# ISAE-PNX/SaDVIO

Measured on AMD Instinct MI355X. Metric: BA iterations/sec (ms/solve in ms_per_solve), 20-KF/8k-landmark window, higher is better.
Workload: dtype f64; 1 GPU; synthetic 20 KF x 8000 landmarks x 40000 reprojection factors (pixel), GN 10 iters (LM step attempts, early exits disabled); windows_per_gpu=1, parallelism=single window, n_kf=20, n_lmk=8000, n_obs=40000, reduced_dim=114

## Files before the change

### sadvio_amd/csrc/kernels.h

```cpp
#pragma once
#include "ba_types.h"
#include "device_math.h"
#include "chol16.h"

namespace sadvio {

struct DevPtrs {
    const WinDev* win;
    const Tile* tiles;
    const double* kf_T0;
    const int* kf_fidx;
    double* xp; double* xv; double* xba; double* xbg;
    long long xp_stride, xv_stride, xl_stride;
    const double* kf_vel; const double* kf_ba; const double* kf_bg;
    const double* cam_K; const double* cam_T; const double* cam_isig;
    const double* lmk_p; double* xl; double* s_lmk;
    const unsigned char* lmk_const;
    const int* lmk_ob; const int* lmk_oe;
    const int* obs_kf; const int* obs_cam; const double* obs_meas;
    const unsigned char* obs_slot;
    const int* tile_kf;
    const int* tile_lmk;
    const int* tile_row;
    const int4* pre_lane;
// ... 260 lines not shown

struct ObsLin {
    double r[2], Jp[12], Jl[6];
    double rho;
    int row;
    int slot;
    bool valid;
    bool counted;
};

struct ObsPre {
    int slot, craw;
    double m[3];
};
template <int FACTOR>
__device__ __forceinline__ ObsPre obs_prefetch(const DevPtrs& P, int o) {
    ObsPre q;
    q.slot = P.obs_slot[o];
    q.craw = P.obs_cam[o];
    if (FACTOR == 0) { const double* m = P.obs_meas + 2 * (long long)o; q.m[0] = m[0]; q.m[1] = m[1]; q.m[2] = 0.0; }
    else { const double* m = P.obs_meas + 3 * (long long)o; q.m[0] = m[0]; q.m[1] = m[1]; q.m[2] = m[2]; }
    return q;
}

template <int FACTOR, bool RARE>
__device__ __forceinline__ void lane_linearize(const DevPtrs& P, const double* poseTab, const double* camTab,
                                               const int* rowTab, int cam_base, const ObsPre& ob, const double* pw, bool keep_jl,
                                               bool lcounted, ObsLin& L) {
    const int slot = ob.slot;
    const int craw = ob.craw;
    const int cam = craw < 0 ? 0 : craw - cam_base;
    const double* tab = poseTab + slot * POSE_TAB;
    const double* ct = camTab + cam * 17;
    L.slot = slot;
    L.row = rowTab[slot];
    if (RARE && craw < 0) {
        const int code = -1 - craw;
        const SparseDev& f = P.sparse[code >> 1];
        p2l_pseudo_obs<true>(tab, pw, f.delta, f.W, code & 1, L.r, L.Jp, L.Jl);
        L.rho = L.r[0] * L.r[0] + L.r[1] * L.r[1];
        if (L.row < 0) {
#pragma unroll
            for (int i = 0; i < 12; i++) L.Jp[i] = 0.0;
        }
        if (!keep_jl) {
#pragma unroll
            for (int i = 0; i < 6; i++) L.Jl[i] = 0.0;
        }
        L.counted = (L.row >= 0) || lcounted;
        return;
    }
    if (FACTOR == 0) {
        pixel_factor<true>(tab, ct, ct + 4, pw, ob.m[0], ob.m[1], ct[16], L.r, L.Jp, L.Jl);
    } else {
        double b[3] = {ob.m[0], ob.m[1], ob.m[2]};
        angular_factor<true>(tab, ct + 4, pw, b, ct[16], L.r, L.Jp, L.Jl);
    }
    L.rho = L.r[0] * L.r[0] + L.r[1] * L.r[1];
    if (RARE) {
        double sc;
        L.rho = huber_rho(P.o.huber_a, L.rho, sc);
        if (sc != 1.0) {
            L.r[0] *= sc; L.r[1] *= sc;
#pragma unroll
            for (int i = 0; i < 12; i++) L.Jp[i] *= sc;
#pragma unroll
            for (int i = 0; i < 6; i++) L.Jl[i] *= sc;
        }
    }
    if (L.row < 0) {
#pragma unroll
        for (int i = 0; i < 12; i++) L.Jp[i] = 0.0;
    }
    if (!keep_jl) {
#pragma unroll
        for (int i = 0; i < 6; i++) L.Jl[i] = 0.0;
    }
    L.counted = (L.row >= 0) || lcounted;
    if (!L.counted) {  }
}

__device__ __forceinline__ bool group_eliminate(const DevPtrs& P, const ObsLin& L, int G, int gl, bool lmk_valid,
                                                bool lfree, int nobs, double radius, bool write_scale, bool leader,
                                                double* Mi, double* g) {
    double H[6];
    H[0] = L.Jl[0] * L.Jl[0] + L.Jl[3] * L.Jl[3];
    H[1] = L.Jl[0] * L.Jl[1] + L.Jl[3] * L.Jl[4];
    H[2] = L.Jl[0] * L.Jl[2] + L.Jl[3] * L.Jl[5];
    H[3] = L.Jl[1] * L.Jl[1] + L.Jl[4] * L.Jl[4];
    H[4] = L.Jl[1] * L.Jl[2] + L.Jl[4] * L.Jl[5];
    H[5] = L.Jl[2] * L.Jl[2] + L.Jl[5] * L.Jl[5];
    g[0] = L.Jl[0] * L.r[0] + L.Jl[3] * L.r[1];
    g[1] = L.Jl[1] * L.r[0] + L.Jl[4] * L.r[1];
    g[2] = L.Jl[2] * L.r[0] + L.Jl[5] * L.r[1];
#pragma unroll
    for (int i = 0; i < 6; i++) H[i] = group_sum(H[i], G);
#pragma unroll
    for (int i = 0; i < 3; i++) g[i] = group_sum(g[i], G);
    const bool active = lmk_valid && lfree && nobs > 0;
    if (!active) {
#pragma unroll
        for (int i = 0; i < 6; i++) Mi[i] = 0.0;
        return false;
    }
    double s[3];
    if (write_scale) {
        s[0] = P.o.jacobi_scaling ? 1.0 / (1.0 + sqrt(H[0])) : 1.0;
        s[1] = P.o.jacobi_scaling ? 1.0 / (1.0 + sqrt(H[3])) : 1.0;
        s[2] = P.o.jacobi_scaling ? 1.0 / (1.0 + sqrt(H[5])) : 1.0;
        if (leader) {
            P.s_lmk[3 * (long long)gl] = s[0]; P.s_lmk[3 * (long long)gl + 1] = s[1]; P.s_lmk[3 * (long long)gl + 2] = s[2];
        }
    } else {
        s[0] = P.s_lmk[3 * (long long)gl]; s[1] = P.s_lmk[3 * (long long)gl + 1]; s[2] = P.s_lmk[3 * (long long)gl + 2];
    }
    const double ir = 1.0 / radius;
    const double s0 = s[0] * s[0], s1 = s[1] * s[1], s2 = s[2] * s[2];
    double M[6] = {H[0], H[1], H[2], H[3], H[4], H[5]};
    M[0] += fmin(fmax(s0 * H[0], P.o.min_lm_diagonal), P.o.max_lm_diagonal) * ir / s0;
    M[3] += fmin(fmax(s1 * H[3], P.o.min_lm_diagonal), P.o.max_lm_diagonal) * ir / s1;
    M[5] += fmin(fmax(s2 * H[5], P.o.min_lm_diagonal), P.o.max_lm_diagonal) * ir / s2;
    sym3_chol_inverse(M, Mi);
    return true;
}

__device__ __forceinline__ void stage_tables(const DevPtrs& P, const Tile& T, int buf, double* poseTab, double* camTab,
                                             int* rowTab) {
    const int tid = threadIdx.x;
    const double* src = P.ptab + (long long)buf * P.ptab_stride;
    for (int i = tid; i < T.n_kf * POSE_TAB; i += blockDim.x) {
        const int k = i / POSE_TAB, e = i - k * POSE_TAB;
        poseTab[i] = src[(long long)P.tile_kf[T.kf_off + k] * POSE_TAB + e];
    }
    for (int i = tid; i < T.n_cam * 17; i += blockDim.x) {
        const int c = i / 17, e = i - 17 * c;
        const int gc = T.cam_base + c;
        camTab[i] = e < 4 ? P.cam_K[4 * (long long)gc + e] : (e < 16 ? P.cam_T[12 * (long long)gc + e - 4] : P.cam_isig[gc]);
    }
    for (int i = tid; i < T.n_kf; i += blockDim.x) rowTab[i] = P.tile_row[T.kf_off + i];
}

__device__ __forceinline__ void wave_lds_fence() {
    __builtin_amdgcn_fence(__ATOMIC_RELEASE, "wavefront");
    __builtin_amdgcn_wave_barrier();
    __builtin_amdgcn_fence(__ATOMIC_ACQUIRE, "wavefront");
}

__host__ __device__ inline size_t tile_tables_bytes(int n_kf) {
    size_t b = sizeof(double) * ((size_t)n_kf * POSE_TAB + MAX_WIN_CAM * 17) + sizeof(int) * (size_t)(n_kf > MAX_TILE_KF ? n_kf : MAX_TILE_KF);
    return (b + 15) & ~(size_t)15;
}

__device__ __forceinline__ int tile_landmark(const Tile& T, const int* __restrict__ tile_lmk, int i) { return T.lmk_off >= 0 ? tile_lmk[T.lmk_off + i] : T.lmk0 + i; }

__global__ __launch_bounds__(BUILD_THREADS) void k_pre_packets(const Tile* __restrict__ tiles, const int* __restrict__ lmk_ob, const int* __restrict__ lmk_oe,
                                                               const int* __restrict__ tile_kf, const int* __restrict__ tile_lmk, const int* __restrict__ kf_fidx, int4* __restrict__ pre_lane,
                                                               int2* __restrict__ pre_kf) {
    const Tile T = tiles[blockIdx.x];
    const int tid = threadIdx.x;
    if (tid < BUILD_THREADS / 8) {
        const int lane0 = tid * 8, wv = lane0 >> 6, ln = lane0 & 63;
        const int G = T.G, lpw = 64 / G, grp = ln / G, q0 = ln - grp * G, nl = T.n_lmk;
        const bool valid = wv * lpw + grp < nl;
        const int gl = nl > 0 ? tile_landmark(T, tile_lmk, valid ? wv * lpw + grp : 0) : T.lmk0;
        const int ob = nl > 0 ? lmk_ob[gl] : 0, nobs = (valid && nl > 0) ? lmk_oe[gl] - ob : 0;
        pre_lane[(long long)blockIdx.x * (BUILD_THREADS / 8) + tid] = make_int4(gl, ob, nobs | (valid ? 1 << 16 : 0), q0);
    }
    if (tid < PRE_KF) {
        int2 e = make_int2(-1, -1);
        if (tid < T.n_kf) { e.x = tile_kf[T.kf_off + tid]; e.y = kf_fidx[e.x]; }
        pre_kf[(long long)blockIdx.x * PRE_KF + tid] = e;
    }
}

template <bool COST_ONLY> __device__ __forceinline__ void pose_factor_eval(const DevPtrs& P, int slot, int idx, int ln);
template <int FACTOR, bool RARE, bool IMU>
__global__ __launch_bounds__(BUILD_THREADS, IMU ? 1 : 2) void k_build(DevPtrs P, int slot, int max_tile_kf, int strip_doubles, int Rp) {
    extern __shared__ __attribute__((aligned(16))) char smem[];
    if (IMU && (int)blockIdx.x >= P.n_tiles) {
        pose_factor_eval<false>(P, slot, (int)blockIdx.x - P.n_tiles, threadIdx.x);
        return;
    }
    const Tile T = P.tiles[blockIdx.x];
    const int tid = threadIdx.x, wv = tid >> 6, ln = tid & 63;
    int4 pl = make_int4(0, -1, 0, 0);
    int2 pk = make_int2(-1, -1);
    if (P.pre_lane) {
        pl = P.pre_lane[(long long)blockIdx.x * (BUILD_THREADS / 8) + (tid >> 3)];
        pk = P.pre_kf[(long long)blockIdx.x * PRE_KF + tid / POSE_TAB];
    }
    SADVIO_TS(3, 32);
    SADVIO_WG_TS(3, 0);
    __shared__ double s_part[BUILD_WAVES * 4];
    double* poseTab = (double*)smem;
    double* camTab = poseTab + (size_t)max_tile_kf * POSE_TAB;
    int* rowTab = (int*)(camTab + MAX_WIN_CAM * 17);
    double* stage = (double*)(smem + tile_tables_bytes(max_tile_kf));
    const int G = T.G, lpw = 64 / G;
    const int grp = ln / G, q = ln - grp * G;
    const int nl = T.n_lmk;
    LmState st;
    IterAcc a;
    LmState prev;
    const bool own_decision = !(slot == 0 || P.decide_kernel);
    double pc = 0.0, pm = 0.0, psn = 0.0, pcn = 0.0;
    auto decision_inputs = [&](int dec_w, int t0, int nt) {
        if (!own_decision) {
            st = P.states[(long long)dec_w * P.state_stride + slot];
            return;
        }
        a = P.acc[(long long)dec_w * P.state_stride + slot - 1];
        prev = P.states[(long long)dec_w * P.state_stride + slot - 1];
        if (P.world > 1) {
            if (wv == 0) {
                const double* rs = P.rank_s + (long long)dec_w * P.world * 4;
                for (int r = ln; r < P.world; r += 64) { pc += rs[4 * r]; pm += rs[4 * r + 1]; psn += rs[4 * r + 2]; pcn += rs[4 * r + 3]; }
            }
        } else {
            const TileAcc* ta = P.tacc + (long long)((slot - 1) & 1) * P.n_tiles + t0;
            double v[4][4];
#pragma unroll
            for (int u = 0; u < 4; u++) {
                const int t = tid + u * BUILD_THREADS;
                const bool in = t < nt;
                const TileAcc* e = ta + (in ? t : 0);
                v[u][0] = in ? e->cand_cost : 0.0; v[u][1] = in ? e->mcc : 0.0; v[u][2] = in ? e->step_norm2 : 0.0; v[u][3] = in ? e->cand_norm2 : 0.0;
            }
            pc = (v[0][0] + v[1][0]) + (v[2][0] + v[3][0]); pm = (v[0][1] + v[1][1]) + (v[2][1] + v[3][1]);
            psn = (v[0][2] + v[1][2]) + (v[2][2] + v[3][2]); pcn = (v[0][3] + v[1][3]) + (v[2][3] + v[3][3]);
        }
    };
    if (P.n_win == 1) decision_inputs(0, 0, P.n_tiles);
    else decision_inputs(T.w, T.win_tile0, T.win_ntiles);
    bool first_valid;
    int gl_first, pre_ob, pre_oe, pre_o;
    static_assert(MAX_LMK_OBS <= 0xff, "a first-round packet carries the landmark's observation count in 8 bits");
    if (P.pre_lane) {
        first_valid = (pl.z >> 16) & 1; gl_first = pl.x; pre_ob = pl.y; pre_oe = pl.y + (pl.z & 0xff);
        pre_o = (pl.w + (tid & 7) < (pl.z & 0xff)) ? pl.y + pl.w + (tid & 7) : -1;
    } else {
        first_valid = wv * lpw + grp < nl;
        gl_first = tile_landmark(T, P.tile_lmk, first_valid ? wv * lpw + grp : 0);
        pre_ob = P.lmk_ob[gl_first]; pre_oe = P.lmk_oe[gl_first];
        pre_o = (first_valid && q < pre_oe - pre_ob) ? pre_ob + q : -1;
    }
    const int pre_lcode = P.lmk_const ? P.lmk_const[gl_first] : 0;
    double pre_p[3], pre_x0[3], pre_x1[3];
#pragma unroll
    for (int i = 0; i < 3; i++) {
        pre_p[i] = P.lmk_p[3 * (long long)gl_first + i];
        pre_x0[i] = P.xl[3 * (long long)gl_first + i];
        pre_x1[i] = P.xl[P.xl_stride + 3 * (long long)gl_first + i];
    }
    double pre_t0 = 0.0, pre_t1 = 0.0;
    if (P.pre_lane) {
        if (pk.x >= 0) {
            const long long src = (long long)pk.x * POSE_TAB + (tid - (tid / POSE_TAB) * POSE_TAB);
            pre_t0 = P.ptab[src]; pre_t1 = P.ptab[P.ptab_stride + src];
        }
    } else if (tid < T.n_kf * POSE_TAB) {
        const int k = tid / POSE_TAB, e = tid - k * POSE_TAB;
        const long long src = (long long)P.tile_kf[T.kf_off + k] * POSE_TAB + e;
        pre_t0 = P.ptab[src]; pre_t1 = P.ptab[P.ptab_stride + src];
    }
    for (int i = tid; i < T.n_cam * 17; i += blockDim.x) {
        const int c = i / 17, e = i - 17 * c;
        const int gc = T.cam_base + c;
        camTab[i] = e < 4 ? P.cam_K[4 * (long long)gc + e] : (e < 16 ? P.cam_T[12 * (long long)gc + e - 4] : P.cam_isig[gc]);
    }
    for (int i = tid; i < T.n_kf; i += blockDim.x) rowTab[i] = P.tile_row[T.kf_off + i];
    ObsPre pre_obs;
    pre_obs.slot = 0; pre_obs.craw = 0; pre_obs.m[0] = pre_obs.m[1] = pre_obs.m[2] = 0.0;
    if (pre_o >= 0) pre_obs = obs_prefetch<FACTOR>(P, pre_o);
    if (own_decision) {
        pc = wave_sum(pc); pm = wave_sum(pm); psn = wave_sum(psn); pcn = wave_sum(pcn);
        if (ln == 0) { s_part[wv * 4] = pc; s_part[wv * 4 + 1] = pm; s_part[wv * 4 + 2] = psn; s_part[wv * 4 + 3] = pcn; }
        __syncthreads();
        a.cand_cost += (s_part[0] + s_part[4]) + (s_part[8] + s_part[12]); a.mcc += (s_part[1] + s_part[5]) + (s_part[9] + s_part[13]);
        a.step_norm2 += (s_part[2] + s_part[6]) + (s_part[10] + s_part[14]); a.cand_norm2 += (s_part[3] + s_part[7]) + (s_part[11] + s_part[15]);
        st = lm_decide(prev, a, P.o);
        __syncthreads();
        if (T.first_of_window && tid == 0) { P.states[(long long)T.w * P.state_stride + slot] = st; trace_write(P, T.w, slot - 1, prev, a, st); }
    }
    if (st.done) return;
    SADVIO_TS(3, 33);
    double* Stile = stage + BUILD_WAVES * strip_doubles;
    const int Nt = 6 * T.n_free;
    const int tri_n = Nt * (Nt + 1) / 2;
    double* gT = Stile + tri_n;
    double* gfT = gT + Nt;
    double* hdT = gfT + Nt;
    const bool lds_mode = T.lds_mode != 0;
    if (tid < T.n_kf * POSE_TAB) poseTab[tid] = st.cur ? pre_t1 : pre_t0;
    {
        const double* src = P.ptab + (long long)st.cur * P.ptab_stride;
        for (int i = tid + blockDim.x; i < T.n_kf * POSE_TAB; i += blockDim.x) {
            const int k = i / POSE_TAB, e = i - k * POSE_TAB;
            poseTab[i] = src[(long long)P.tile_kf[T.kf_off + k] * POSE_TAB + e];
        }
    }
    if (lds_mode) {
        const int nz = tri_n + 3 * Nt;
        for (int i = tid; i < nz; i += blockDim.x) Stile[i] = 0.0;
    }
    __syncthreads();

    SADVIO_TS(3, 34);
    double* Sg = P.S + T.S_off;
    double* gredg = P.gred + T.red_off;
    double* gfullg = P.gfull + T.red_off;
    double* hdg = P.hdiag + T.red_off;
    const int dpf = T.dpf, Np = T.Np;
    const double* xl = P.xl + (long long)st.cur * P.xl_stride;
    double* wstage = stage + wv * strip_doubles;
    const bool gemm_mode = T.lds_mode == 2;
    double cost_part = 0.0, fixed_part = 0.0, gmax_part = 0.0;
    typedef double d4 __attribute__((ext_vector_type(4)));
    d4 accs[3] = {(d4){0.0, 0.0, 0.0, 0.0}, (d4){0.0, 0.0, 0.0, 0.0}, (d4){0.0, 0.0, 0.0, 0.0}};
    for (int base = wv * lpw; base < nl; base += BUILD_WAVES * lpw) {
        const int lm = base + grp;
        const bool lmk_valid = lm < nl;
        const bool first = base == wv * lpw;
        const int gl = first ? gl_first : tile_landmark(T, P.tile_lmk, lmk_valid ? lm : 0);
        const int ob = first ? pre_ob : P.lmk_ob[gl], oe = first ? pre_oe : P.lmk_oe[gl];
        const int nobs = lmk_valid ? oe - ob : 0;
        const int lcode = first ? pre_lcode : (P.lmk_const ? P.lmk_const[gl] : 0);
        const bool lfree = lcode == 0;
        ObsLin L;
        L.valid = q < nobs;
        L.row = -1; L.slot = 0; L.counted = false;
        if (L.valid) {
            double pw[3];
            ObsPre obq;
            if (first) {
#pragma unroll
                for (int i = 0; i < 3; i++) pw[i] = pre_p[i] + (st.cur ? pre_x1[i] : pre_x0[i]);
                obq = pre_obs;
            } else {
#pragma unroll
                for (int i = 0; i < 3; i++) pw[i] = P.lmk_p[3 * (long long)gl + i] + xl[3 * (long long)gl + i];
                obq = obs_prefetch<FACTOR>(P, ob + q);
            }
            lane_linearize<FACTOR, RARE>(P, poseTab, camTab, rowTab, T.cam_base, obq, pw, lfree, lcode != 1, L);
            const double c = L.rho;
            if (L.counted) cost_part += c;
            else { fixed_part += c; L.r[0] = 0.0; L.r[1] = 0.0; }
        } else {
            L.r[0] = L.r[1] = 0.0;
#pragma unroll
            for (int i = 0; i < 12; i++) L.Jp[i] = 0.0;
#pragma unroll
            for (int i = 0; i < 6; i++) L.Jl[i] = 0.0;
        }
    SADVIO_TS(3, 35);
        double Mi[6], g[3];
        const bool active = group_eliminate(P, L, G, gl, lmk_valid, lfree, nobs, st.radius, slot == 0, q == 0, Mi, g);
        if (active && q == 0) gmax_part = fmax(gmax_part, fmax(fabs(g[0]), fmax(fabs(g[1]), fabs(g[2]))));
    SADVIO_TS(3, 36);
        double N[6], gam[3];
        li_row(Mi, L.Jl[0], L.Jl[1], L.Jl[2], N);
        li_row(Mi, L.Jl[3], L.Jl[4], L.Jl[5], N + 3);
        li_vec(Mi, g, gam);
        if (gemm_mode) {
            constexpr int Kw = 32, KS = Kw + 2;
            double* Yb = wstage;
            const double* Eb = Yb;
            {
                double2* z = (double2*)wstage;
                const double2 zero2 = make_double2(0.0, 0.0);
                for (int i = ln; i < Rp * KS / 2; i += 64) z[i] = zero2;
            }
            const bool vrow = L.valid && L.row >= 0;
            const int myrow = vrow ? L.row : -2 - ln;
            const int row_prev = dpp_i32<0x111>(myrow);
            const int row_next = dpp_i32<0x101>(myrow);
            const bool follower = vrow && q > 0 && row_prev == myrow;
            const bool has_follower = vrow && q + 1 < G && row_next == myrow;
            const int row_next2 = RARE ? dpp_i32<0x102>(myrow) : -1;
            const bool has_follower2 = RARE && vrow && q + 2 < G && row_next2 == myrow;
            const bool head = vrow && !follower;
            const double rt0 = L.r[0] - (N[0] * gam[0] + N[1] * gam[1] + N[2] * gam[2]);
            const double rt1 = L.r[1] - (N[3] * gam[0] + N[4] * gam[1] + N[5] * gam[2]);
            wave_lds_fence();
    SADVIO_TS(3, 37);
#pragma unroll
            for (int i = 0; i < 6; i++) {
                const double j0 = vrow ? L.Jp[i] : 0.0, j1 = vrow ? L.Jp[6 + i] : 0.0;
                double y[3];
#pragma unroll
                for (int c = 0; c < 3; c++) {
                    y[c] = j0 * N[c] + j1 * N[3 + c];
                    const double yn = dpp_f64<0x101>(y[c]);
                    if (has_follower) y[c] += yn;
                    if (RARE) {
                        const double yn2 = dpp_f64<0x102>(y[c]);
                        if (has_follower2) y[c] += yn2;
                    }
                }
                if (head) {
                    double2* yp = (double2*)(Yb + (myrow + i) * KS + 4 * grp);
                    yp[0] = make_double2(y[0], y[1]); yp[1] = make_double2(y[2], 0.0);
                }
            }
            wave_lds_fence();
    SADVIO_TS(3, 38);
            {
                const int lr = ln & 15, lk = ln >> 4;
                const int nt16 = (Nt + 15) >> 4;
#pragma unroll
                for (int pp = 0; pp < 3; pp++) {
                    const int tr = pp < 1 ? 0 : 1, tc = pp - tr;
                    if (tr < nt16) {
                        d4& loc = accs[pp];
                        double av[8], bv[8];
#pragma unroll
                        for (int kk = 0; kk < 8; kk++) {
                            const int k = (4 * kk < Kw) ? 4 * kk + lk : lk;
                            av[kk] = Yb[(16 * tr + lr) * KS + k];
                            bv[kk] = Eb[(16 * tc + lr) * KS + k];
                        }
#pragma unroll
                        for (int kk = 0; kk < 8; kk++)
                            if (4 * kk < Kw) loc = __builtin_amdgcn_mfma_f64_16x16x4f64(av[kk], bv[kk], loc, 0, 0, 0);
                    }
                }
            }
            {
#ifdef SADVIO_KERNEL_TS
                {
                    const int rowu = vrow ? L.row : -1;
                    const int mism = (dpp_i32<0x128>(rowu) != rowu) | (xor16_other(rowu) != rowu) | (xor32_other(rowu) != rowu);
                    const bool uniform = (G == 8) && (__ballot(mism) == 0ull);
                    const int nheads = __popcll(__ballot(head));
                    if ((P.debug & 4096) && slot == 3 && blockIdx.x < DBG_WG_MAX && ln == 0) {
                        atomicMax((int*)&P.dbg_ts[DBG_WG_BASE + 4 * blockIdx.x + 3], nheads);
                        if (uniform) atomicAdd((int*)&P.dbg_ts[DBG_WG_BASE + 4 * blockIdx.x + 3] + 1, 1);
                    }
                }
#endif
// ... 435 lines not shown
                                              double* r, double* J) {
    const int fi = f.kf >= 0 ? P.kf_fidx[f.kf] : -1;
    const int lr0 = sparse_lr0(P, W, f);
    const int lr1 = (f.lmk1 >= 0 && P.lmk_red) ? P.lmk_red[f.lmk1] : -1;
    if (fi < 0 && lr0 < 0 && lr1 < 0) return false;
    const int dpf = W.dpf;
    if (f.type == 5) {
        double da[6], db[6];
        for (int q = 0; q < 6; q++) {
            da[q] = xp[6 * (long long)f.kf + q] + ((y && fi >= 0) ? y[fi * dpf + q] : 0.0);
            db[q] = xp[6 * (long long)f.kf2 + q] + ((y && lr0 >= 0) ? y[lr0 + q] : 0.0);
        }
        relative_pose_factor(P.kf_T0 + 12 * (long long)f.kf, P.kf_T0 + 12 * (long long)f.kf2, f.T_prior, f.W, da, db, r, J);
        return true;
    }
    if (f.type == 0) {
        double prm[15];
        const long long k = f.kf;
        for (int q = 0; q < 6; q++) prm[q] = xp[6 * k + q] + ((y && fi >= 0) ? y[fi * dpf + q] : 0.0);
        for (int q = 0; q < 3; q++) {
            const bool st = y && fi >= 0 && dpf == 15;
            prm[6 + q] = xv[3 * k + q] + (st ? y[fi * 15 + 6 + q] : 0.0);
            prm[9 + q] = xba[3 * k + q] + (st ? y[fi * 15 + 9 + q] : 0.0);
            prm[12 + q] = xbg[3 * k + q] + (st ? y[fi * 15 + 12 + q] : 0.0);
        }
        if (INL) imu_prior_factor_body(P.kf_T0 + 12 * k, P.kf_vel + 3 * k, P.kf_ba + 3 * k, P.kf_bg + 3 * k, f.T_prior, f.v_prior,
                                       f.ba_prior, f.bg_prior, f.W, prm, r, J);
        else imu_prior_factor(P.kf_T0 + 12 * k, P.kf_vel + 3 * k, P.kf_ba + 3 * k, P.kf_bg + 3 * k, f.T_prior, f.v_prior,
                              f.ba_prior, f.bg_prior, f.W, prm, r, J);
        return true;
    }
    double q0[3], q1[3] = {0.0, 0.0, 0.0};
    for (int a = 0; a < 3; a++) {
        q0[a] = P.lmk_p[3 * (long long)f.lmk0 + a] + xl[3 * (long long)f.lmk0 + a] + ((y && lr0 >= 0) ? y[lr0 + a] : 0.0);
        if (f.type == 3) q1[a] = P.lmk_p[3 * (long long)f.lmk1 + a] + xl[3 * (long long)f.lmk1 + a] + ((y && lr1 >= 0) ? y[lr1 + a] : 0.0);
    }
    if (f.type == 1) {
        double d6[6];
        for (int q = 0; q < 6; q++) d6[q] = xp[6 * (long long)f.kf + q] + ((y && fi >= 0) ? y[fi * dpf + q] : 0.0);
        pose_to_landmark_factor(P.kf_T0 + 12 * (long long)f.kf, q0, f.delta, f.W, d6, r, J);
        return true;
    }
    double e[3];
    for (int a = 0; a < 3; a++) e[a] = q0[a] - q1[a] - f.delta[a];
    m3_vec(f.W, e, r);
    if (J) {
        for (int i = 0; i < 3; i++)
            for (int j = 0; j < 3; j++) { J[i * 15 + j] = f.W[3 * i + j]; J[i * 15 + 3 + j] = -f.W[3 * i + j]; }
    }
    return true;
}

__device__ __noinline__ bool sparse_eval(const DevPtrs& P, const WinDev& W, const SparseDev& f, const double* xp, const double* xv,
                                        const double* xba, const double* xbg, const double* xl, const double* y,
                                        double* r, double* J) {
    return sparse_eval_t<false>(P, W, f, xp, xv, xba, xbg, xl, y, r, J);
}


__device__ __forceinline__ double prior_lin_record(const double* T0, const double* Tp, const double* inf, const double* d6, double* rec) {
    double r[6], J[36];
    pose_prior_factor(T0, Tp, inf, d6, r, J);
    double c = 0.0;
#pragma unroll
    for (int a = 0; a < 6; a++) {
        c += r[a] * r[a];
        double g = 0.0;
#pragma unroll
        for (int q = 0; q < 6; q++) g += J[6 * q + a] * r[q];
        rec[a] = g;
#pragma unroll
        for (int b = 0; b <= a; b++) {
            double hh = 0.0;
#pragma unroll
            for (int q = 0; q < 6; q++) hh += J[6 * q + a] * J[6 * q + b];
            rec[6 + a * (a + 1) / 2 + b] = hh;
        }
    }
    rec[27] = c;
    return c;
}

__device__ __noinline__ void pose_table_store(const double* T0, double d0, double d1, double d2, double d3, double d4, double d5, double* dst) {
    double T0r[12], tab[POSE_TAB];
#pragma unroll
    for (int i = 0; i < 12; i++) T0r[i] = T0[i];
    const double d6[6] = {d0, d1, d2, d3, d4, d5};
    pose_table_entry(T0r, d6, tab);
#pragma unroll
    for (int i = 0; i < POSE_TAB; i++) dst[i] = tab[i];
}
__device__ __noinline__ double prior_lin_record_call(const double* T0, double d0, double d1, double d2, double d3, double d4, double d5, const PriorDev* pr,
                                                     double* rec) {
    double T0r[12];
#pragma unroll
    for (int i = 0; i < 12; i++) T0r[i] = T0[i];
    const double d6[6] = {d0, d1, d2, d3, d4, d5};
    const PriorDev q = *pr;
    return prior_lin_record(T0r, q.T_prior, q.inf, d6, rec);
}

template <int MODE, bool EXTRAS>
__global__ __launch_bounds__(SOLVE_THREADS) void k_solve(DevPtrs P, int slot) {
    extern __shared__ __attribute__((aligned(16))) char smem[];
    constexpr bool BIG = MODE != 0;
    const int w = blockIdx.x;
    const WinDev W = P.win[w];
    if (BIG != (W.ld != 0)) return;
    const int tid = threadIdx.x;
    const int wv = __builtin_amdgcn_readfirstlane(tid >> 6), ln = tid & 63, nwv = blockDim.x >> 6;
    LmState* stp = P.states + (long long)w * P.state_stride + slot;
    IterAcc* acc = P.acc + (long long)w * P.state_stride + slot;
    __shared__ int s_done;
    __shared__ double s_red[SOLVE_THREADS / 64 * 4];
    SADVIO_TS(3, 0);
#ifdef SADVIO_KERNEL_TS
    if ((P.debug & 4096) && blockIdx.x == 0 && tid == 0 && slot == 3) P.dbg_ts[20] = clock64();
#endif
    LmState st = *stp;
    if (MODE == 1 && tid == 0) P.big_info[w] = 0;
    if (st.done) return;
    const int Np = W.Np;
    const long long ld = W.ld;
    double* Sg = P.S + W.S_off;
    double* gredg = P.gred + W.red_off;
    double* gfullg = P.gfull + W.red_off;
    double* hdg = P.hdiag + W.red_off;
    const int nbt = c16_blocks(Np + 1);
    const int img_n = c16_size(Np);
    double* A = BIG ? Sg : (double*)smem;
    double* y = BIG ? gredg : A + img_n;
    double* gf = BIG ? gfullg : y + Np;
    double* hd = BIG ? hdg : gf + Np;
    double* xs = BIG ? gredg : hd + Np;
    double* pub = xs + Np + (Np & 1);
    double* yv = pub + C16_WORK;
    double* kfc = yv + 16 * nbt;
    auto aidx = [&](int i, int j) -> long long { return BIG ? (long long)i * ld + j : (long long)c16_index(i, j); };
    const int cur = st.cur;
    const double* xp = P.xp + (long long)cur * P.xp_stride;
    const int n_imu = W.imu_end - W.imu_begin;
    double early_cost = 0.0, early_fixed = 0.0, early_gm = 0.0;
    double cost_part = 0.0, fixed_part = 0.0;
    const int n_pri = W.prior_end - W.prior_begin;
    const double* plin = P.prior_lin + (long long)cur * P.prior_lin_stride + (long long)W.prior_begin * PRIOR_LIN;
    double pl_v = 0.0;
    int pl_fi = -1;
    if (MODE != 2 && tid < n_pri * 28) {
        const int p = tid / 28, e = tid - 28 * p;
        pl_v = plin[p * PRIOR_LIN + e];
        pl_fi = P.kf_fidx[P.priors[W.prior_begin + p].kf];
    }
    double* sp = P.s_pose + W.red_off;
    double c_sp = 1.0;
    const bool det = P.world > 1;
    if (MODE != 2) {
    double im_ix[8], im_v[8];
    const int n_imu_items = (EXTRAS && !det && !P.imu_direct) ? n_imu * IMU_NE : 0;
    if (EXTRAS) {
#pragma unroll
        for (int u = 0; u < 8; u++) {
            const int it = tid + u * (int)blockDim.x;
            im_ix[u] = -1.0; im_v[u] = 0.0;
            if (it < n_imu_items) {
                const int k = it / IMU_NE, e = it - IMU_NE * k;
                const double* row = P.imu_scratch + (long long)cur * P.imu_scratch_stride + (long long)(W.imu_begin + k) * IMU_ROW;
// ... 230 lines not shown
        } else {
            cost_part += pc[0];
            pc[0] = 0.0;
        }
    }
    double gm = early_gm;
    cost_part += early_cost; fixed_part += early_fixed;
    __syncthreads();
    if (!BIG) {
        if (tid < Np) {
            gm = fmax(gm, fabs(gf[tid]));
            const double hdi = hd[tid];
            double s = c_sp;
            if (slot == 0) { s = P.o.jacobi_scaling ? 1.0 / (1.0 + sqrt(hdi)) : 1.0; sp[tid] = s; }
            const double s2 = s * s;
            A[c16_index(tid, tid)] += fmin(fmax(s2 * hdi, P.o.min_lm_diagonal), P.o.max_lm_diagonal) / st.radius / s2;
            A[c16_index(Np, tid)] = y[tid];
        }
    } else {
        for (int i = tid; i < Np; i += blockDim.x) gm = fmax(gm, fabs(gf[i]));
    }
    gm = wave_max(gm); cost_part = wave_sum(cost_part); fixed_part = wave_sum(fixed_part);
    if (ln == 0) { s_red[wv * 3] = gm; s_red[wv * 3 + 1] = cost_part; s_red[wv * 3 + 2] = fixed_part; }
    if (tid == 0) s_done = 0;
    __syncthreads();
    if (!BIG) c16_symmetrize(A, nbt);
    if (tid == blockDim.x - 1) {
        double g = 0, cs = 0, fs = 0;
        for (int k = 0; k < nwv; k++) { g = fmax(g, s_red[k * 3]); cs += s_red[k * 3 + 1]; fs += s_red[k * 3 + 2]; }
        acc->gmax_bits = (unsigned long long)__double_as_longlong(g);
        acc->lin_cost = cs;
        acc->fixed_cost = fs;
        acc->cand_cost = 0.0; acc->mcc = 0.0; acc->step_norm2 = 0.0; acc->cand_norm2 = 0.0;
        const bool time_up = P.o.max_time_ticks > 0.0 && P.t_start && (double)(wall_clock64() - *P.t_start) >= P.o.max_time_ticks;
        acc->time_up = time_up ? 1 : 0;
        const bool no_iterations = st.iter == 0 && P.o.max_num_iterations <= 0;
        if (time_up || g <= P.o.gradient_tolerance || no_iterations) {
            LmState e = st;
            e.done = 1; e.termination = (time_up || g > P.o.gradient_tolerance) ? 0 : 3;
            e.x_cost = 0.5 * cs;
            if (e.iter == 0) e.initial_cost = e.x_cost;
            *stp = e;
            s_done = 1;
        }
    }
    __syncthreads();
    if (s_done) return;
    SADVIO_TS(3, 2);
    if (BIG) {
        for (int i = tid; i < Np; i += blockDim.x) {
            double s;
            if (slot == 0) { s = P.o.jacobi_scaling ? 1.0 / (1.0 + sqrt(hd[i])) : 1.0; sp[i] = s; }
            else s = sp[i];
            double s2 = s * s;
            A[aidx(i, i)] += fmin(fmax(s2 * hd[i], P.o.min_lm_diagonal), P.o.max_lm_diagonal) / st.radius / s2;
        }
        __syncthreads();
    }
    SADVIO_TS(3, 3);
    if (MODE == 1) return;
    }
    long long* ts = SADVIO_TS_PTR((P.debug & 4096) && blockIdx.x == 0 && slot == 3);
    if (MODE == 0) {
        bool ok = true;
        if (Np > 0) ok = c16_solve<1>(A, Np, xs, pub, yv, ts ? ts + 64 : nullptr, nullptr, P.c16_old_tail != 0);
        if (!ok) {
            if (tid == 0) acc->chol_fail = 1;
            return;
        }
    } else {
        y = P.delta + W.red_off;
        if (P.big_info[w] != 0) {
            for (int i = tid; i < Np; i += blockDim.x) { gredg[i] = 0.0; gfullg[i] = 0.0; hdg[i] = 0.0; }
            if (tid == 0) acc->chol_fail = 1;
            return;
        }
    }
    SADVIO_TS(3, 4);
    double* dl = P.delta + W.red_off;
    double sn = 0.0, cn = 0.0;
    bool bad = false;
    for (int i = tid; i < Np; i += blockDim.x) {
        double d = -xs[i];
        dl[i] = d;
        y[i] = d;
        sn += d * d;
        if (!isfinite(d)) bad = true;
        if (BIG) { gredg[i] = 0.0; gfullg[i] = 0.0; hdg[i] = 0.0; }
    }
    __syncthreads();
    SADVIO_TS(3, 5);
    double* xpc = P.xp + (long long)(1 - cur) * P.xp_stride;
    for (int k = tid; k < W.n_kf; k += blockDim.x) {
        int g = W.kf_base + k;
        const bool pre = MODE == 0 && k < SOLVE_KFC;
        const double* kc = kfc + (pre ? k : 0) * SOLVE_KFC_STRIDE;
        int fi = pre ? (int)kc[0] : P.kf_fidx[g];
        double d6[6];
        const double* T0r = pre ? kc + 7 : P.kf_T0 + 12 * (long long)g;
        double vbb[9];
        if (W.dpf == 15) {
            const double* xs3[3] = {P.xv + (long long)cur * P.xv_stride, P.xba + (long long)cur * P.xv_stride, P.xbg + (long long)cur * P.xv_stride};
#pragma unroll
            for (int q = 0; q < 3; q++)
#pragma unroll
                for (int i = 0; i < 3; i++) vbb[3 * q + i] = pre ? kc[19 + 3 * q + i] : xs3[q][3 * (long long)g + i];
        }
#pragma unroll
        for (int i = 0; i < 6; i++) {
            double v = (pre ? kc[1 + i] : xp[6 * (long long)g + i]) + (fi < 0 ? 0.0 : y[fi * W.dpf + i]);
            xpc[6 * (long long)g + i] = v;
            d6[i] = v;
            if (fi >= 0) cn += v * v;
        }
        pose_table_store(T0r, d6[0], d6[1], d6[2], d6[3], d6[4], d6[5], P.ptab + (long long)(1 - cur) * P.ptab_stride + (long long)g * POSE_TAB);
        if (W.dpf == 15) {
            double* xs3[3] = {P.xv + (long long)(1 - cur) * P.xv_stride, P.xba + (long long)(1 - cur) * P.xv_stride, P.xbg + (long long)(1 - cur) * P.xv_stride};
#pragma unroll
            for (int q = 0; q < 3; q++)
#pragma unroll
                for (int i = 0; i < 3; i++) {
                    const double v = vbb[3 * q + i] + (fi < 0 ? 0.0 : y[fi * 15 + 6 + 3 * q + i]);
                    xs3[q][3 * (long long)g + i] = v;
                    if (fi >= 0) cn += v * v;
                }
        }
    }
    if (EXTRAS && W.line_end > W.line_begin) {
        const double* xlc = P.xline + (long long)cur * P.xline_stride;
        double* xln = P.xline + (long long)(1 - cur) * P.xline_stride;
        for (int it = tid; it < (W.line_end - W.line_begin) * 6; it += blockDim.x) {
            const int l = W.line_begin + it / 6, q = it % 6;
            const int lc = P.lines[l].col;
            const double v = xlc[6 * (long long)l + q] + (lc < 0 ? 0.0 : y[lc + q]);
            xln[6 * (long long)l + q] = v;
            if (lc >= 0) cn += v * v;
        }
    }
    SADVIO_TS(3, 6);
    double mcc = 0.0, cc = 0.0;
    {
        const double* plx = P.prior_lin + (long long)cur * P.prior_lin_stride + (long long)W.prior_begin * PRIOR_LIN;
        double* plc = P.prior_lin + (long long)(1 - cur) * P.prior_lin_stride + (long long)W.prior_begin * PRIOR_LIN;
        for (int p = (int)blockDim.x - 1 - tid; p < W.prior_end - W.prior_begin; p += blockDim.x) {
            const PriorDev* prp = P.priors + W.prior_begin + p;
            const int pkf = prp->kf;
            const int fi = P.kf_fidx[pkf];
            if (fi < 0) continue;
            double d[6], d6[6];
#pragma unroll
            for (int i = 0; i < 6; i++) { d[i] = y[fi * W.dpf + i]; d6[i] = xp[6 * (long long)pkf + i] + d[i]; }
            double lin = 0.0, quad = 0.0;
#pragma unroll
            for (int a = 0; a < 6; a++) {
                lin += d[a] * plx[p * PRIOR_LIN + a];
#pragma unroll
                for (int b = 0; b <= a; b++) quad += (a == b ? 0.5 : 1.0) * d[a] * d[b] * plx[p * PRIOR_LIN + 6 + a * (a + 1) / 2 + b];
            }
            mcc += -(lin + quad);
            cc += prior_lin_record_call(P.kf_T0 + 12 * (long long)pkf, d6[0], d6[1], d6[2], d6[3], d6[4], d6[5], prp, plc + p * PRIOR_LIN);
        }
    }
    if (EXTRAS && n_imu > 0) {
        const double* xv = P.xv + (long long)cur * P.xv_stride;
        const double* xba = P.xba + (long long)cur * P.xv_stride;
        const double* xbg = P.xbg + (long long)cur * P.xv_stride;
        const int t0 = blockDim.x > 128 ? 64 : 0;
        for (int it = tid - t0; it >= 0 && it < n_imu * 15; it += blockDim.x - t0) {
            const int k = it / 15, q = it - 15 * k;
            const double* sc = P.imu_scratch + (long long)cur * P.imu_scratch_stride + (long long)(W.imu_begin + k) * IMU_ROW;
            const int fi = (int)sc[IMU_META], fj = (int)sc[IMU_META + 1];
            if (fi < 0 && fj < 0) continue;
            double m = 0.0, r;
            if (q < 9) {
                double jr[24];
#pragma unroll
                for (int a = 0; a < 24; a++) jr[a] = sc[q * 24 + a];
                r = sc[9 * 24 + q];
#pragma unroll
                for (int a = 0; a < 24; a++) { const int ca = imu_col(a, fi, fj); if (ca >= 0) m += jr[a] * y[ca]; }
            } else {
                const int e = q - 9, ax = e % 3, gy = e / 3;
                const double sgm = sc[IMU_META + 2 + gy];
                r = sc[IMU_J + e];
                if (fi >= 0) m -= sgm * y[fi * 15 + 9 + 3 * gy + ax];
                if (fj >= 0) m += sgm * y[fj * 15 + 9 + 3 * gy + ax];
            }
            mcc += -m * (r + 0.5 * m);
        }
    }
    if (EXTRAS && W.spl_end > W.spl_begin) {
        const int t0 = blockDim.x > 320 ? 256 : 0;
        for (int it = tid - t0; it >= 0 && it < (W.spl_end - W.spl_begin) * 15; it += blockDim.x - t0) {
            const int kl = it / 15, q = it - 15 * kl;
            const double* sc = P.sp_scratch + (long long)cur * P.sp_scratch_stride + (long long)P.sp_list[W.spl_begin + kl] * SPARSE_J;
            if (q >= (int)sc[SPARSE_COL + 15]) continue;
            double jr[15], cd[15];
#pragma unroll
            for (int a = 0; a < 15; a++) { jr[a] = sc[q * 15 + a]; cd[a] = sc[SPARSE_COL + a]; }
            const double r = sc[225 + q];
            double m = 0.0;
#pragma unroll
            for (int a = 0; a < 15; a++) { const int ca = (int)cd[a]; if (ca >= 0) m += jr[a] * y[ca]; }
            mcc += -m * (r + 0.5 * m);
        }
    }
    if (EXTRAS && W.lobs_end > W.lobs_begin) {
        const int rows = W.factor_type == 0 ? 4 : 2;
        for (int it = tid; it < (W.lobs_end - W.lobs_begin) * 4; it += blockDim.x) {
            const int k = it >> 2, q = it & 3;
            if (q >= rows) continue;
            const LineObsDev& ob = P.lobs[W.lobs_begin + k];
            const int fi = P.kf_fidx[ob.kf], lc = P.lines[ob.line].col;
            if (fi < 0 && lc < 0) continue;
            const double* sc = P.line_scratch + (long long)(W.lobs_begin + k) * LINE_ROW;
            double m = 0.0;
            for (int a = 0; a < 6; a++) {
                if (fi >= 0) m += sc[q * 12 + a] * y[fi * W.dpf + a];
                if (lc >= 0) m += sc[q * 12 + 6 + a] * y[lc + a];
            }
            mcc += -m * (sc[48 + q] + 0.5 * m);
        }
    }
    SADVIO_TS(3, 7);
    sn = wave_sum(sn); cn = wave_sum(cn); mcc = wave_sum(mcc); cc = wave_sum(cc);
    if (bad) acc->chol_fail = 1;
    __syncthreads();
    if (ln == 0) { s_red[wv * 4] = sn; s_red[wv * 4 + 1] = cn; s_red[wv * 4 + 2] = mcc; s_red[wv * 4 + 3] = cc; }
    __syncthreads();
    if (tid == 0) {
        double a0 = 0, a1 = 0, a2 = 0, a3 = 0;
        for (int k = 0; k < nwv; k++) { a0 += s_red[k * 4]; a1 += s_red[k * 4 + 1]; a2 += s_red[k * 4 + 2]; a3 += s_red[k * 4 + 3]; }
        acc->step_norm2 = a0; acc->cand_norm2 = a1; acc->mcc = a2; acc->cand_cost = a3;
    }
    SADVIO_TS(3, 8);
    if (ts && tid == 0) { ts[15] = wall_clock64(); ts[21] = clock64(); }
}


__device__ __forceinline__ void zero_s_slice(const DevPtrs& P, const Tile& T, int tile_index) {
    if (T.ld != 0) return;
    const int n2 = c16_size(T.Np) >> 1;
    const int per = (n2 + T.win_ntiles - 1) / T.win_ntiles;
    const int i0 = (tile_index - T.win_tile0) * per, i1 = min(i0 + per, n2);
    double2* S2 = (double2*)(P.S + T.S_off);
    const double2 z2 = make_double2(0.0, 0.0);
    for (int i = i0 + (int)threadIdx.x; i < i1; i += blockDim.x) S2[i] = z2;
}

template <int FACTOR, bool RARE, bool IMU>
__global__ __launch_bounds__(BUILD_THREADS) void k_backsub(DevPtrs P, int slot, int max_tile_kf) {
    extern __shared__ __attribute__((aligned(16))) char smem[];
    if (IMU && (int)blockIdx.x >= P.n_tiles) {
        if (threadIdx.x < 64) pose_factor_eval<true>(P, slot, (int)blockIdx.x - P.n_tiles, threadIdx.x);
        return;
    }
    const Tile T = P.tiles[blockIdx.x];
    const int tid = threadIdx.x, wv = tid >> 6, ln = tid & 63;
    int4 pl = make_int4(0, -1, 0, 0);
    int2 pk = make_int2(-1, -1), pk6 = make_int2(-1, -1);
    if (P.pre_lane) {
        pl = P.pre_lane[(long long)blockIdx.x * (BUILD_THREADS / 8) + (tid >> 3)];
        pk = P.pre_kf[(long long)blockIdx.x * PRE_KF + tid / POSE_TAB];
        if (tid < PRE_KF * 6) pk6 = P.pre_kf[(long long)blockIdx.x * PRE_KF + tid / 6];
    }
    LmState st;
    int chol_fail;
    if (P.n_win == 1) { st = P.states[slot]; chol_fail = P.acc[slot].chol_fail; }
    else { st = P.states[(long long)T.w * P.state_stride + slot]; chol_fail = P.acc[(long long)T.w * P.state_stride + slot].chol_fail; }
    zero_s_slice(P, T, blockIdx.x);
    double* poseTab = (double*)smem;
    double* camTab = poseTab + (size_t)max_tile_kf * POSE_TAB;
    int* rowTab = (int*)(camTab + MAX_WIN_CAM * 17);
    double* candTab = (double*)(smem + tile_tables_bytes(max_tile_kf));
    double* dpTab = candTab + (size_t)max_tile_kf * 12;
    const int G = T.G, lpw = 64 / G;
    const int grp = ln / G, q = ln - grp * G;
    const int nl = T.n_lmk;
    bool first_valid;
    int gl_first, pre_ob, pre_oe, pre_o;
    static_assert(MAX_LMK_OBS <= 0xff, "a first-round packet carries the landmark's observation count in 8 bits");
    if (P.pre_lane) {
        first_valid = (pl.z >> 16) & 1; gl_first = pl.x; pre_ob = pl.y; pre_oe = pl.y + (pl.z & 0xff);
        pre_o = (pl.w + (tid & 7) < (pl.z & 0xff)) ? pl.y + pl.w + (tid & 7) : -1;
    } else {
        first_valid = wv * lpw + grp < nl;
        gl_first = tile_landmark(T, P.tile_lmk, first_valid ? wv * lpw + grp : 0);
        pre_ob = P.lmk_ob[gl_first]; pre_oe = P.lmk_oe[gl_first];
        pre_o = (first_valid && q < pre_oe - pre_ob) ? pre_ob + q : -1;
    }
    const int pre_lcode = P.lmk_const ? P.lmk_const[gl_first] : 0;
    double pre_p[3], pre_xa[3], pre_xb[3];
#pragma unroll
    for (int i = 0; i < 3; i++) {
        pre_p[i] = P.lmk_p[3 * (long long)gl_first + i];
        pre_xa[i] = P.xl[3 * (long long)gl_first + i];
        pre_xb[i] = P.xl[P.xl_stride + 3 * (long long)gl_first + i];
    }
    ObsPre pre_obs;
    pre_obs.slot = 0; pre_obs.craw = 0; pre_obs.m[0] = pre_obs.m[1] = pre_obs.m[2] = 0.0;
    if (pre_o >= 0) pre_obs = obs_prefetch<FACTOR>(P, pre_o);
    double pre_t0 = 0.0, pre_t1 = 0.0;
    const bool pre_tab = P.pre_lane != nullptr;
    if (pre_tab && pk.x >= 0) {
        const long long src = (long long)pk.x * POSE_TAB + (tid - (tid / POSE_TAB) * POSE_TAB);
        pre_t0 = P.ptab[src]; pre_t1 = P.ptab[P.ptab_stride + src];
    }
    if (st.done || chol_fail) {
        if (tid == 0) {
            TileAcc* ta = P.tacc + (long long)(slot & 1) * P.n_tiles + blockIdx.x;
            ta->cand_cost = 0.0; ta->mcc = 0.0; ta->step_norm2 = 0.0; ta->cand_norm2 = 0.0;
        }
        return;
    }
    const int cur = st.cur;
    const double* xl = P.xl + (long long)cur * P.xl_stride;
    double* xlc = P.xl + (long long)(1 - cur) * P.xl_stride;
    double pre_x[3];
#pragma unroll
    for (int i = 0; i < 3; i++) pre_x[i] = cur ? pre_xb[i] : pre_xa[i];
    if (pre_tab) {
        const double* src = P.ptab + (long long)cur * P.ptab_stride;
        const double* srcc = P.ptab + (long long)(1 - cur) * P.ptab_stride;
        if (tid < T.n_kf * POSE_TAB) {
            const int k = tid / POSE_TAB, e = tid - k * POSE_TAB;
            poseTab[tid] = cur ? pre_t1 : pre_t0;
            if (e < 12) candTab[k * 12 + e] = cur ? pre_t0 : pre_t1;
        }
        for (int i = tid + blockDim.x; i < T.n_kf * POSE_TAB; i += blockDim.x) {
            const int k = i / POSE_TAB, e = i - k * POSE_TAB;
            const long long o = (long long)P.tile_kf[T.kf_off + k] * POSE_TAB + e;
            poseTab[i] = src[o];
            if (e < 12) candTab[k * 12 + e] = srcc[o];
        }
        for (int i = tid; i < T.n_cam * 17; i += blockDim.x) {
            const int c = i / 17, e = i - 17 * c;
            const int gc = T.cam_base + c;
            camTab[i] = e < 4 ? P.cam_K[4 * (long long)gc + e] : (e < 16 ? P.cam_T[12 * (long long)gc + e - 4] : P.cam_isig[gc]);
        }
        for (int i = tid; i < T.n_kf; i += blockDim.x) rowTab[i] = P.tile_row[T.kf_off + i];
        const double* dp = P.delta + T.red_off;
        for (int i = tid; i < T.n_kf * 6; i += blockDim.x) {
            const int k = i / 6, e = i - 6 * k;
            const int fi = (i < PRE_KF * 6) ? pk6.y : P.kf_fidx[P.tile_kf[T.kf_off + k]];
            dpTab[i] = fi < 0 ? 0.0 : dp[fi * T.dpf + e];
        }
    } else {
        stage_tables(P, T, cur, poseTab, camTab, rowTab);
        const double* src = P.ptab + (long long)(1 - cur) * P.ptab_stride;
        for (int i = tid; i < T.n_kf * 12; i += blockDim.x) {
            const int k = i / 12, e = i - 12 * k;
            candTab[i] = src[(long long)P.tile_kf[T.kf_off + k] * POSE_TAB + e];
        }
        const double* dp = P.delta + T.red_off;
        for (int i = tid; i < T.n_kf * 6; i += blockDim.x) {
            const int k = i / 6, e = i - 6 * k;
            const int fi = P.kf_fidx[P.tile_kf[T.kf_off + k]];
            dpTab[i] = fi < 0 ? 0.0 : dp[fi * T.dpf + e];
        }
    }
    __syncthreads();
    double sn = 0.0, cn = 0.0, mcc = 0.0, cc = 0.0;
    for (int base = wv * lpw; base < nl; base += BUILD_WAVES * lpw) {
        const int lm = base + grp;
        const bool lmk_valid = lm < nl;
        const bool first = base == wv * lpw;
        const int gl = first ? gl_first : tile_landmark(T, P.tile_lmk, lmk_valid ? lm : 0);
        const int ob = first ? pre_ob : P.lmk_ob[gl], oe = first ? pre_oe : P.lmk_oe[gl];
        const int nobs = lmk_valid ? oe - ob : 0;
        const int lcode = first ? pre_lcode : (P.lmk_const ? P.lmk_const[gl] : 0);
        const bool lfree = lcode == 0;
        double p0[3], x0[3];
#pragma unroll
        for (int i = 0; i < 3; i++) {
            p0[i] = first ? pre_p[i] : P.lmk_p[3 * (long long)gl + i];
            x0[i] = first ? pre_x[i] : xl[3 * (long long)gl + i];
        }
        ObsLin L;
        L.valid = q < nobs;
        L.row = -1; L.slot = 0; L.counted = false;
        ObsPre obq = pre_obs;
        if (L.valid) {
            const double pw[3] = {p0[0] + x0[0], p0[1] + x0[1], p0[2] + x0[2]};
            if (!first) obq = obs_prefetch<FACTOR>(P, ob + q);
            lane_linearize<FACTOR, RARE>(P, poseTab, camTab, rowTab, T.cam_base, obq, pw, lcode != 1, lcode != 1, L);
            if (!L.counted) { L.r[0] = 0.0; L.r[1] = 0.0; }
        } else {
            L.r[0] = L.r[1] = 0.0;
#pragma unroll
            for (int i = 0; i < 12; i++) L.Jp[i] = 0.0;
#pragma unroll
            for (int i = 0; i < 6; i++) L.Jl[i] = 0.0;
        }
        double Mi[6], g[3];
        const bool active = group_eliminate(P, L, G, gl, lmk_valid, lfree, nobs, st.radius, false, false, Mi, g);

        double e0 = L.r[0], e1 = L.r[1];
        const double* d = dpTab + L.slot * 6;
        if (L.valid && L.row >= 0) {
#pragma unroll
            for (int i = 0; i < 6; i++) { e0 += L.Jp[i] * d[i]; e1 += L.Jp[6 + i] * d[i]; }
        }
        const double tt[3] = {group_sum(L.Jl[0] * e0 + L.Jl[3] * e1, G), group_sum(L.Jl[1] * e0 + L.Jl[4] * e1, G),
                              group_sum(L.Jl[2] * e0 + L.Jl[5] * e1, G)};
        double ut[3], vt3[3];
        li_vec(Mi, tt, ut);
        li_tvec(Mi, ut, vt3);
        double d0 = -vt3[0], d1 = -vt3[1], d2 = -vt3[2];
        if (RARE && lcode == 2) {
            const double* dr = P.delta + T.red_off + P.lmk_red[gl];
            d0 = dr[0]; d1 = dr[1]; d2 = dr[2];
        }
        const double c0 = x0[0] + d0, c1 = x0[1] + d1, c2 = x0[2] + d2;
        if (lmk_valid && q == 0) {
            xlc[3 * (long long)gl] = c0; xlc[3 * (long long)gl + 1] = c1; xlc[3 * (long long)gl + 2] = c2;
            if (active) {
                sn += d0 * d0 + d1 * d1 + d2 * d2;
                cn += c0 * c0 + c1 * c1 + c2 * c2;
            } else if (RARE && lcode == 2 && (P.world == 1 || P.rank == 0)) cn += c0 * c0 + c1 * c1 + c2 * c2;
        }
        if (L.valid && L.counted) {
            const double m0 = (e0 - L.r[0]) + L.Jl[0] * d0 + L.Jl[1] * d1 + L.Jl[2] * d2;
            const double m1 = (e1 - L.r[1]) + L.Jl[3] * d0 + L.Jl[4] * d1 + L.Jl[5] * d2;
            mcc += -m0 * (L.r[0] + 0.5 * m0) - m1 * (L.r[1] + 0.5 * m1);
            const int craw = obq.craw;
            const int cam = craw < 0 ? 0 : craw - T.cam_base;
            const double* ct = camTab + cam * 17;
            const double pw[3] = {p0[0] + c0, p0[1] + c1, p0[2] + c2};
            const double* ctab = candTab + L.slot * 12;
            double r[2];
            if (RARE && craw < 0) {
                const int code = -1 - craw;
                const SparseDev& f = P.sparse[code >> 1];
                p2l_pseudo_obs<false>(ctab, pw, f.delta, f.W, code & 1, r, nullptr, nullptr);
                cc += r[0] * r[0] + r[1] * r[1];
            } else {
            if (FACTOR == 0) {
                pixel_factor<false>(ctab, ct, ct + 4, pw, obq.m[0], obq.m[1], ct[16], r, nullptr, nullptr);
            } else {
                double bb[3] = {obq.m[0], obq.m[1], obq.m[2]};
                angular_factor<false>(ctab, ct + 4, pw, bb, ct[16], r, nullptr, nullptr);
            }
            double sc_unused;
            cc += RARE ? huber_rho(P.o.huber_a, r[0] * r[0] + r[1] * r[1], sc_unused) : r[0] * r[0] + r[1] * r[1];
            }
        }
    }
    sn = wave_sum(sn); cn = wave_sum(cn); mcc = wave_sum(mcc); cc = wave_sum(cc);
    __shared__ double s_part[BUILD_WAVES * 4];
    if (ln == 0) { s_part[wv * 4] = cc; s_part[wv * 4 + 1] = mcc; s_part[wv * 4 + 2] = sn; s_part[wv * 4 + 3] = cn; }
    __syncthreads();
    if (tid == 0) {
        double a0 = 0.0, a1 = 0.0, a2 = 0.0, a3 = 0.0;
        for (int k = 0; k < BUILD_WAVES; k++) { a0 += s_part[k * 4]; a1 += s_part[k * 4 + 1]; a2 += s_part[k * 4 + 2]; a3 += s_part[k * 4 + 3]; }
        TileAcc* ta = P.tacc + (long long)(slot & 1) * P.n_tiles + blockIdx.x;
        ta->cand_cost = a0; ta->mcc = a1; ta->step_norm2 = a2; ta->cand_norm2 = a3;
    }
}

constexpr int DP_LDS_N = 2048;
__device__ __forceinline__ double* dp_ptr(const DevPtrs& P, const WinDev& W, int which) {
    const size_t nf = W.dp_n_full, n = W.dp_n;
    double* D = P.dp_data + W.dp_off;
    switch (which) {
        case 0: return D;
        case 1: return D + nf * n;
        case 2: return D + 2 * nf * n;
        case 3: return D + 2 * nf * n + n * n;
        case 4: return D + 2 * nf * n + n * n + nf;
        case 5: return D + 2 * nf * n + n * n + nf + n;
        case 6: return D + 2 * nf * n + n * n + 2 * nf + n;
        default: return D + 2 * nf * n + n * n + 2 * nf + n + 2;
    }
}

__global__ __launch_bounds__(256) void k_prior_r(DevPtrs P, int slot) {
    const int w = blockIdx.y;
    const WinDev W = P.win[w];
// ... 953 lines not shown
```

Before: 19030 BA iterations/s.

## Prefetch landmark scales and stage pose tables in LDS during solve update

Landmark Jacobi scales are now loaded early, before the linearization, and passed into the elimination, so their global-load latency overlaps other work. In the solve kernel's MODE 0 path, the first keyframes' pose tables are computed from LDS-resident data into an LDS buffer. They are then copied to global memory after the reduction barrier by the threads not on the reduction, and the dl write-back is deferred the same way. This aims to take global stores and latency off the critical path, at the cost of extra register pressure and an added LDS staging pass.

Result: faster. 19310 BA iterations/s, median of 6 (+1.5%).

```diff
diff --git a/sadvio_amd/csrc/kernels.h b/sadvio_amd/csrc/kernels.h
--- a/sadvio_amd/csrc/kernels.h
+++ b/sadvio_amd/csrc/kernels.h
@@ -366,7 +366,7 @@
 
 __device__ __forceinline__ bool group_eliminate(const DevPtrs& P, const ObsLin& L, int G, int gl, bool lmk_valid,
                                                 bool lfree, int nobs, double radius, bool write_scale, bool leader,
-                                                double* Mi, double* g) {
+                                                double* Mi, double* g, const double* s_pre) {
     double H[6];
     H[0] = L.Jl[0] * L.Jl[0] + L.Jl[3] * L.Jl[3];
     H[1] = L.Jl[0] * L.Jl[1] + L.Jl[3] * L.Jl[4];
@@ -395,6 +395,8 @@
         if (leader) {
             P.s_lmk[3 * (long long)gl] = s[0]; P.s_lmk[3 * (long long)gl + 1] = s[1]; P.s_lmk[3 * (long long)gl + 2] = s[2];
         }
+    } else if (s_pre) {
+        s[0] = s_pre[0]; s[1] = s_pre[1]; s[2] = s_pre[2];
     } else {
         s[0] = P.s_lmk[3 * (long long)gl]; s[1] = P.s_lmk[3 * (long long)gl + 1]; s[2] = P.s_lmk[3 * (long long)gl + 2];
     }
@@ -535,6 +537,11 @@
         pre_p[i] = P.lmk_p[3 * (long long)gl_first + i];
         pre_x0[i] = P.xl[3 * (long long)gl_first + i];
         pre_x1[i] = P.xl[P.xl_stride + 3 * (long long)gl_first + i];
+    }
+    double pre_s[3] = {1.0, 1.0, 1.0};
+    if (slot != 0) {
+#pragma unroll
+        for (int i = 0; i < 3; i++) pre_s[i] = P.s_lmk[3 * (long long)gl_first + i];
     }
     double pre_t0 = 0.0, pre_t1 = 0.0;
     if (P.pre_lane) {
@@ -610,6 +617,11 @@
         const int nobs = lmk_valid ? oe - ob : 0;
         const int lcode = first ? pre_lcode : (P.lmk_const ? P.lmk_const[gl] : 0);
         const bool lfree = lcode == 0;
+        double sc[3] = {pre_s[0], pre_s[1], pre_s[2]};
+        if (!first && slot != 0) {
+#pragma unroll
+            for (int i = 0; i < 3; i++) sc[i] = P.s_lmk[3 * (long long)gl + i];
+        }
         ObsLin L;
         L.valid = q < nobs;
         L.row = -1; L.slot = 0; L.counted = false;
@@ -638,7 +650,7 @@
         }
     SADVIO_TS(3, 35);
         double Mi[6], g[3];
-        const bool active = group_eliminate(P, L, G, gl, lmk_valid, lfree, nobs, st.radius, slot == 0, q == 0, Mi, g);
+        const bool active = group_eliminate(P, L, G, gl, lmk_valid, lfree, nobs, st.radius, slot == 0, q == 0, Mi, g, sc);
         if (active && q == 0) gmax_part = fmax(gmax_part, fmax(fabs(g[0]), fmax(fabs(g[1]), fabs(g[2]))));
     SADVIO_TS(3, 36);
         double N[6], gam[3];
@@ -1240,6 +1252,16 @@
 }
 
 __device__ __noinline__ void pose_table_store(const double* T0, double d0, double d1, double d2, double d3, double d4, double d5, double* dst) {
+    double T0r[12], tab[POSE_TAB];
+#pragma unroll
+    for (int i = 0; i < 12; i++) T0r[i] = T0[i];
+    const double d6[6] = {d0, d1, d2, d3, d4, d5};
+    pose_table_entry(T0r, d6, tab);
+#pragma unroll
+    for (int i = 0; i < POSE_TAB; i++) dst[i] = tab[i];
+}
+typedef __attribute__((address_space(3))) double lds_double;
+__device__ __noinline__ void pose_table_lds(const lds_double* T0, double d0, double d1, double d2, double d3, double d4, double d5, lds_double* dst) {
     double T0r[12], tab[POSE_TAB];
 #pragma unroll
     for (int i = 0; i < 12; i++) T0r[i] = T0[i];
@@ -1636,7 +1658,7 @@
     bool bad = false;
     for (int i = tid; i < Np; i += blockDim.x) {
         double d = -xs[i];
-        dl[i] = d;
+        if (MODE != 0) dl[i] = d;
         y[i] = d;
         sn += d * d;
         if (!isfinite(d)) bad = true;
@@ -1645,24 +1667,60 @@
     __syncthreads();
     SADVIO_TS(3, 5);
     double* xpc = P.xp + (long long)(1 - cur) * P.xp_stride;
-    for (int k = tid; k < W.n_kf; k += blockDim.x) {
+    const int n_park = MODE == 0 ? min(W.n_kf, SOLVE_KFC) : 0;
+    const bool tab_lds = MODE == 0 && n_park * POSE_TAB <= img_n;
+    if (MODE == 0 && tid < n_park) {
+        const int k = tid, g = W.kf_base + k;
+        const lds_double* kc = (const lds_double*)(kfc + k * SOLVE_KFC_STRIDE);
+        const lds_double* yl = (const lds_double*)y;
+        const int fi = (int)kc[0];
+        const bool dpf15 = W.dpf == 15;
+        double d6[6], vbb[9], dy[15];
+#pragma unroll
+        for (int i = 0; i < 6; i++) d6[i] = kc[1 + i];
+#pragma unroll
+        for (int i = 0; i < 6; i++) dy[i] = fi < 0 ? 0.0 : yl[fi * W.dpf + i];
+        if (dpf15) {
+#pragma unroll
+            for (int i = 0; i < 9; i++) { vbb[i] = kc[19 + i]; dy[6 + i] = fi < 0 ? 0.0 : yl[fi * 15 + 6 + i]; }
+        }
+#pragma unroll
+        for (int i = 0; i < 6; i++) {
+            d6[i] += dy[i];
+            if (fi >= 0) cn = fma(d6[i], d6[i], cn);
+        }
+        if (tab_lds) pose_table_lds(kc + 7, d6[0], d6[1], d6[2], d6[3], d6[4], d6[5], (lds_double*)A + k * POSE_TAB);
+        else pose_table_store(kfc + k * SOLVE_KFC_STRIDE + 7, d6[0], d6[1], d6[2], d6[3], d6[4], d6[5], P.ptab + (long long)(1 - cur) * P.ptab_stride + (long long)g * POSE_TAB);
+#pragma unroll
+        for (int i = 0; i < 6; i++) xpc[6 * (long long)g + i] = d6[i];
+        if (dpf15) {
+            double* xs3[3] = {P.xv + (long long)(1 - cur) * P.xv_stride, P.xba + (long long)(1 - cur) * P.xv_stride, P.xbg + (long long)(1 - cur) * P.xv_stride};
+#pragma unroll
+            for (int q = 0; q < 3; q++)
+#pragma unroll
+                for (int i = 0; i < 3; i++) {
+                    const double v = vbb[3 * q + i] + dy[6 + 3 * q + i];
+                    xs3[q][3 * (long long)g + i] = v;
+                    if (fi >= 0) cn = fma(v, v, cn);
+                }
+        }
+    }
+    for (int k = (MODE == 0 ? SOLVE_KFC : 0) + tid; k < W.n_kf; k += blockDim.x) {
         int g = W.kf_base + k;
-        const bool pre = MODE == 0 && k < SOLVE_KFC;
-        const double* kc = kfc + (pre ? k : 0) * SOLVE_KFC_STRIDE;
-        int fi = pre ? (int)kc[0] : P.kf_fidx[g];
+        int fi = P.kf_fidx[g];
         double d6[6];
-        const double* T0r = pre ? kc + 7 : P.kf_T0 + 12 * (long long)g;
+        const double* T0r = P.kf_T0 + 12 * (long long)g;
         double vbb[9];
         if (W.dpf == 15) {
             const double* xs3[3] = {P.xv + (long long)cur * P.xv_stride, P.xba + (long long)cur * P.xv_stride, P.xbg + (long long)cur * P.xv_stride};
 #pragma unroll
             for (int q = 0; q < 3; q++)
 #pragma unroll
-                for (int i = 0; i < 3; i++) vbb[3 * q + i] = pre ? kc[19 + 3 * q + i] : xs3[q][3 * (long long)g + i];
+                for (int i = 0; i < 3; i++) vbb[3 * q + i] = xs3[q][3 * (long long)g + i];
         }
 #pragma unroll
         for (int i = 0; i < 6; i++) {
-            double v = (pre ? kc[1 + i] : xp[6 * (long long)g + i]) + (fi < 0 ? 0.0 : y[fi * W.dpf + i]);
+            double v = xp[6 * (long long)g + i] + (fi < 0 ? 0.0 : y[fi * W.dpf + i]);
             xpc[6 * (long long)g + i] = v;
             d6[i] = v;
             if (fi >= 0) cn += v * v;
@@ -1782,6 +1840,14 @@
     __syncthreads();
     if (ln == 0) { s_red[wv * 4] = sn; s_red[wv * 4 + 1] = cn; s_red[wv * 4 + 2] = mcc; s_red[wv * 4 + 3] = cc; }
     __syncthreads();
+    if (MODE == 0) {
+        const int t0 = nwv > 1 ? 64 : 0, nth = (int)blockDim.x - t0;
+        if (tab_lds) {
+            double* pt = P.ptab + (long long)(1 - cur) * P.ptab_stride + (long long)W.kf_base * POSE_TAB;
+            for (int i = tid - t0; i >= 0 && i < n_park * POSE_TAB; i += nth) pt[i] = A[i];
+        }
+        for (int i = tid - t0; i >= 0 && i < Np; i += nth) dl[i] = y[i];
+    }
     if (tid == 0) {
         double a0 = 0, a1 = 0, a2 = 0, a3 = 0;
         for (int k = 0; k < nwv; k++) { a0 += s_red[k * 4]; a1 += s_red[k * 4 + 1]; a2 += s_red[k * 4 + 2]; a3 += s_red[k * 4 + 3]; }
@@ -1947,7 +2013,7 @@
             for (int i = 0; i < 6; i++) L.Jl[i] = 0.0;
         }
         double Mi[6], g[3];
-        const bool active = group_eliminate(P, L, G, gl, lmk_valid, lfree, nobs, st.radius, false, false, Mi, g);
+        const bool active = group_eliminate(P, L, G, gl, lmk_valid, lfree, nobs, st.radius, false, false, Mi, g, nullptr);
 
         double e0 = L.r[0], e1 = L.r[1];
         const double* d = dpTab + L.slot * 6;
```
